# RyanXLi/OneshotDet

Hardware: AMD Instinct MI355X
Metric: images/sec/GPU fwd+bwd, 800x1024 target + 127x127 query, bs=8; 1->8 GPU scaling (higher is better)
Workload: dtype bf16; 1 GPU; BASELINE.json configs[2]: bs=8/GPU, 800x1024 target + 127x127 query, bf16 MFMA convs, forward (two R-50-FPN backbones, query pooling, correlation, FCOS head, training proposals) + FCOS loss + backward (stem/layer1 frozen) + gradient all-reduce + SGD(momentum) + weight repack; global_batch=8, parallelism=dp1: one rank, no collective anywhere in the step, world_size=1

## Files before the change

### oneshotdet_amd/_lib.py

```python
import ctypes as C
import os

_HERE = os.path.dirname(os.path.abspath(__file__))
LIB_PATH = os.environ.get("OSD_LIB_PATH") or os.path.join(_HERE, "lib", "liboneshotdet_hip.so")

OSD_F32, OSD_BF16 = 0, 1
ABI_VERSION = 4
ACT_NONE, ACT_RELU, ACT_EXP_SCALE = 0, 1, 2
RES_NONE, RES_SAME, RES_UP2X, RES_DOWN2X = 0, 1, 2, 3
GN_SPLITS = 64


class ConvDesc(C.Structure):
    _fields_ = [(n, C.c_int32) for n in (
        "dtype", "n", "h", "w", "cin", "in_stride_n", "in_stride_h", "in_stride_w", "ho", "wo", "cout", "r", "s",
        "stride_h", "stride_w", "pad_h", "pad_w", "w_rows", "out_stride", "res_mode", "res_h", "res_w", "res_stride",
        "act")] + [("act_scale", C.c_float), ("relu_in", C.c_int32), ("algo", C.c_int32), ("reserved0", C.c_int32),
                   ("ordered_ws", C.c_void_p), ("ordered_ws_bytes", C.c_int64)]


_p, _i, _f, _i64 = C.c_void_p, C.c_int, C.c_float, C.c_int64

SIGNATURES = {
    "osd_last_error_string": (C.c_char_p, []),
# ... 85 lines not shown
    "osd_box_loss": (_i, [_p, _p, _p, _p, _i, _i, _i, _f, _f, _p, _p, _i, _i, _p]),
    "osd_voc_match": (_i, [_p, _p, _p, _p, _p, _p, _p, _p, _i, _i, _i, _f, _p, _p, _p]),
    "osd_voc_curves": (_i, [_p, _p, _p, _i, _p, _p, _p]),
    "osd_voc_ap": (_i, [_p, _p, _p, _p, _p, _i, _i, _p, _p]),
    "osd_coco_match": (_i, [_p, _p, _p, _p, _p, _p, _i, _i, _i, _p, _i, _p, _i, _p, _p, _p, _p]),
    "osd_groupnorm_act_rois_bwd": (_i, [_p, _p, _p, _p, _p, _p, _p, _p, _p, _i, _i, _i, _i, _f, _f, _i, _i, _i, _i, _p]),
    "osd_rois_sum": (_i, [_p, _p, _i, _i, _i64, _i, _p]),
    "osd_roi_pool_levels_bwd": (_i, [_i, _p, _p, _p, _p, _p, _p, _p, _i, _i, _i, _i, _i, _i, _i, _p]),
    "osd_image_transform": (_i, [_p, _i, _i, _i, _i, _i, _i, _p, _p, _p, _i, _i, _i, _i, _i, _i, _i, _p, _p]),
    "osd_image_transform_workspace_bytes": (_i64, [_i, _i, _i, _i]),
    "osd_image_transform_batch": (_i, [_i, _p, _p, _p, _p, _p, _p, _i, _p, _p, _p, _i, _i, _i, _i, _i, _i, _i, _p, _p]),
}

BOX_CLS_CE, BOX_CLS_FOCAL, BOX_CLS_MSE = 0, 1, 2
SIGNATURES_BOX_MODES = {
    "osd_box_loss_opt": (_i, [_p, _p, _p, _p, _i, _i, _i, _f, _f, _p, _p, _i, _i, _i, _f, _f, _p]),
    "osd_box_decode_opt": (_i, [_p, _p, _p, _p, _p, _p, _p, _i, _i, _i, _i, _p, _f, _f, _p, _f, _i, _i, _p]),
}

BOX_CLS_L1, BOX_CLS_CXE = 3, 4
SOFT_LABEL_DISCRETE, SOFT_LABEL_LINEAR, SOFT_LABEL_TRANS_LINEAR, SOFT_LABEL_TRANS_4TH_LINEAR = 0, 1, 2, 3
SIGNATURES_SOFT_LABELS = {
    "osd_box_match_sample_soft": (_i, [_p, _p, _p, _p, _p, _p, _i, _i, _i, _i, _f, _f, _p, _p, _p, _p, _p, _p, _p, _p, _i, _p, _p, _p]),
    "osd_box_loss_soft": (_i, [_p, _p, _p, _p, _i, _i, _i, _f, _f, _p, _p, _i, _i, _p, _i, _p]),
}

SIGNATURES_NEG_SUPPORT = {
    "osd_box_loss_neg_support": (_i, [_p, _p, _p, _p, _p, _i, _i, _i, _f, _f, _f, _f, _p, _p, _p, _i, _i, _p]),
}

SIGNATURES_SOLVER = {
    "osd_solver_set": (_i, [_p, _f, _i, _p]),
    "osd_sgd_momentum_multi_dev": (_i, [_p, _p, _i, _p, _p, _p, _p, _f, _p]),
    "osd_sgd_momentum_pack_multi_dev": (_i, [_p, _p, _i, _p, _p, _p, _p, _p, _i, _p, _f, _i, _p]),
}

SIGNATURES_CLASS_SWEEP = {
    "osd_class_sweep_group": (_i, []),
    "osd_correlate_levels_sweep": (_i, [_i, _p, _p, _p, _p, _i, _i, _i, _i, _p]),
    "osd_roi_pool_levels_sweep": (_i, [_i, _p, _p, _p, _p, _p, _p, _p, _i, _i, _i, _i, _i, _i, _i, _p, _i, _p]),
}

SIGNATURES_GALLERY = {
    "osd_correlate_levels_gallery": (_i, [_i, _p, _p, _p, _p, _p, _i, _i, _i, _i, _i, _p]),
    "osd_groupnorm_act_rois_gallery": (_i, [_p, _p, _p, _p, _p, _p, _i, _i, _i, _i, _f, _f, _i, _i, _i, _i, _i, _p]),
}

PRED_BWD_BOTH, PRED_BWD_DGRAD, PRED_BWD_WGRAD = 0, 1, 2
SIGNATURES_PRED_BWD = {
    "osd_pred_bwd_workspace_bytes": (_i64, [_i, _p, _p, _p, _i, _i]),
    "osd_conv2d_pred_bwd": (_i, [C.POINTER(ConvDesc), _i, _p, _p, _p, _p, _p, _p, _p, _p, _p, _p, _i, _p]),
}

_lib = None


class OsdError(RuntimeError):
    pass


def load():
    global _lib
    if _lib is not None:
        return _lib
    if not os.path.exists(LIB_PATH):
        raise OsdError("liboneshotdet_hip.so not built (%s missing): run `python -m oneshotdet_amd.build` or "
                       "__graft_entry__.build(); there is no CPU/eager fallback" % LIB_PATH)
    import torch
    lib = C.CDLL(LIB_PATH)
    for name, (res, args) in (list(SIGNATURES.items()) + list(SIGNATURES_BOX_MODES.items()) + list(SIGNATURES_SOFT_LABELS.items())
                              + list(SIGNATURES_NEG_SUPPORT.items()) + list(SIGNATURES_SOLVER.items())
                              + list(SIGNATURES_CLASS_SWEEP.items()) + list(SIGNATURES_GALLERY.items())
                              + list(SIGNATURES_PRED_BWD.items())):
        fn = getattr(lib, name)
        fn.restype = res
        fn.argtypes = args
    if lib.osd_abi_version() != ABI_VERSION:
        raise OsdError("%s reports ABI %d, this binding is written for ABI %d: rebuild it (`python -m oneshotdet_amd.build`)"
                       % (LIB_PATH, lib.osd_abi_version(), ABI_VERSION))
    _lib = lib
    return lib


def check(rc, what=""):
    if rc != 0:
        msg = load().osd_last_error_string()
        err = OsdError("%s failed (%d): %s" % (what, rc, msg.decode() if msg else "?"))
        err.code = rc
        raise err


def call(name, *args):
    lib = load()
    check(getattr(lib, name)(*args), name)
```

### oneshotdet_amd/build.py

```python
import os
import subprocess
import sys

HERE = os.path.dirname(os.path.abspath(__file__))
CSRC = os.path.join(HERE, "csrc")
LIBDIR = os.path.join(HERE, "lib")
TAG = os.environ.get("OSD_BUILD_TAG", "")
LIB = os.path.join(LIBDIR, "liboneshotdet_hip%s.so" % ("_" + TAG if TAG else ""))
SOURCES = ["osd_error.hip", "conv_igemm.hip", "conv_igemm_dma.hip", "conv_igemm_sp.hip", "conv_pred.hip", "conv_pred_bwd.hip", "conv_px.hip", "conv_wgrad.hip", "conv_wgrad_sk.hip", "backward.hip", "groupnorm_onepass.hip", "loss.hip", "elementwise.hip", "proposals.hip", "box_head.hip", "transforms.hip", "box_train.hip", "evaluation.hip", "query_avgpool.hip", "class_sweep.hip", "gallery.hip"]
HIPCC = os.environ.get("HIPCC", "/opt/rocm/bin/hipcc")
FLAGS = ["--offload-arch=gfx950", "-O3", "-fPIC", "-std=c++17", "-Wno-unused-result"] + os.environ.get("OSD_BUILD_FLAGS", "").split()


def _stale(target, deps):
    if not os.path.exists(target):
        return True
    t = os.path.getmtime(target)
    return any(os.path.getmtime(d) > t for d in deps)


def build_library(force=False, verbose=True):
    os.makedirs(LIBDIR, exist_ok=True)
    objdir = os.path.join(LIBDIR, "obj" + ("_" + TAG if TAG else ""))
    os.makedirs(objdir, exist_ok=True)
    headers = sorted(os.path.join(CSRC, f) for f in os.listdir(CSRC) if f.endswith(".h")) + [os.path.join(os.path.dirname(HERE), "include", h) for h in ("oneshotdet_hip.h", "oneshotdet_hip_box_modes.h", "oneshotdet_hip_soft_labels.h", "oneshotdet_hip_neg_support.h", "oneshotdet_hip_solver.h", "oneshotdet_hip_class_sweep.h", "oneshotdet_hip_gallery.h", "oneshotdet_hip_pred_bwd.h")]
    keep = set(src.replace(".hip", ".o") for src in SOURCES)
    for f in os.listdir(objdir):
        if f.endswith(".o") and f not in keep:
            os.remove(os.path.join(objdir, f))
    objs, procs = [], []
    for src in SOURCES:
        s = os.path.join(CSRC, src)
        o = os.path.join(objdir, src.replace(".hip", ".o"))
        objs.append(o)
        if force or _stale(o, [s] + headers):
            cmd = [HIPCC] + FLAGS + ["-c", s, "-o", o]
            if verbose:
                print(" ".join(cmd), flush=True)
            procs.append((src, subprocess.Popen(cmd, stdout=subprocess.PIPE, stderr=subprocess.STDOUT)))
    for src, p in procs:
        out, _ = p.communicate()
        if p.returncode != 0:
            sys.stderr.write(out.decode())
            raise RuntimeError("hipcc failed on %s" % src)
    if force or procs or _stale(LIB, objs):
        cmd = [HIPCC, "--offload-arch=gfx950", "-shared", "-fPIC", "-o", LIB] + objs
        if verbose:
            print(" ".join(cmd), flush=True)
        subprocess.check_call(cmd)
    return LIB


if __name__ == "__main__":
    print(build_library(force="--force" in sys.argv))
```

### oneshotdet_amd/csrc/backward.hip

```cpp
#include "osd_common.h"
#include "conv_params.h"

namespace {

constexpr int kMaxBlocks = 2048;
inline int grid_for(long long work, int threads) {
  long long b = (work + threads - 1) / threads;
  if (b < 1) b = 1;
  return (int)(b > kMaxBlocks ? kMaxBlocks : b);
}

template <typename T> struct Chunk;
template <> struct Chunk<float> {
  static constexpr int N = 4;
  float v[4];
  __device__ __forceinline__ void load(const float* p) {
    const float4 t = *reinterpret_cast<const float4*>(p);
    v[0] = t.x; v[1] = t.y; v[2] = t.z; v[3] = t.w;
  }
  __device__ __forceinline__ void store(float* p) const { *reinterpret_cast<float4*>(p) = make_float4(v[0], v[1], v[2], v[3]); }
};
template <> struct Chunk<__bf16> {
  static constexpr int N = 8;
  float v[8];
  __device__ __forceinline__ void load(const __bf16* p) {
    const bf16x8 t = *reinterpret_cast<const bf16x8*>(p);
#pragma unroll
    for (int i = 0; i < 8; ++i) v[i] = (float)t[i];
  }
  __device__ __forceinline__ void store(__bf16* p) const {
    bf16x8 t;
#pragma unroll
    for (int i = 0; i < 8; ++i) t[i] = (__bf16)v[i];
    *reinterpret_cast<bf16x8*>(p) = t;
  }
};

template <typename T>
__global__ void pack_dgrad_weight_kernel(const float* __restrict__ w, const float* __restrict__ scale, T* __restrict__ dst,
                                         int cout, int cin, int R, int S, int rows, int cout_pad, int src_orsi) {
  const long long total = (long long)rows * R * S * cout_pad;
  for (long long i = blockIdx.x * (long long)blockDim.x + threadIdx.x; i < total; i += (long long)gridDim.x * blockDim.x) {
    const int co = (int)(i % cout_pad);
    long long t = i / cout_pad;
    const int s = (int)(t % S); t /= S;
    const int r = (int)(t % R);
    const int ci = (int)(t / R);
    float v = 0.f;
    if (co < cout && ci < cin) {
      v = src_orsi ? w[(((size_t)co * R + (R - 1 - r)) * S + (S - 1 - s)) * cin + ci]
                   : w[(((size_t)co * cin + ci) * R + (R - 1 - r)) * S + (S - 1 - s)];
      if (scale) v *= scale[co];
    }
    dst[i] = from_f32<T>(v);
// ... 774 lines not shown
#pragma unroll
        for (int e = 0; e < E; ++e) s[e] += live * a[k].v[e] * bb[k].v[e];
      }
    }
  }
  __shared__ float red[256 * 8];
#pragma unroll
  for (int e = 0; e < E; ++e) red[(pl * cch + cc) * E + e] = (pl < lanes) ? s[e] : 0.f;
  __syncthreads();
  for (int ch = threadIdx.x; ch < c; ch += blockDim.x) {
    float t = 0.f;
    for (int l = 0; l < lanes; ++l) t += red[l * c + ch];
    if (p0 < p1) atomicAdd(dq + (size_t)img * c + ch, t);
  }
}
}

extern "C" int osd_correlate_bwd_query_levels(int n_levels, const void* const* gs, const void* const* feats,
                                              float* const* dqs, const int32_t* hws, int n, int c, int dtype, void* stream) {
  const int e = dtype == OSD_BF16 ? 8 : 4;
  if (n_levels < 1 || n_levels > kCorrQLevels || !gs || !feats || !dqs || !hws || c % e || 256 % (c / e) || c > 2048)
    return osd_fail(OSD_ERR_INVALID_ARG, "correlate_bwd_query_levels: bad args");
  if (dtype != OSD_F32 && dtype != OSD_BF16) return osd_fail(OSD_ERR_INVALID_ARG, "correlate_bwd_query_levels: bad dtype");
  if (n == 0) return OSD_OK;
  CorrQLevels L;
  L.n_levels = 0;
  int blocks = 0;
  for (int i = 0; i < n_levels; ++i)
    if (!dqs[i]) return osd_fail(OSD_ERR_INVALID_ARG, "correlate_bwd_query_levels: null dq at level %d", i);
  for (int i = 0; i < n_levels;) {
    int j = i + 1;
    while (j < n_levels && dqs[j] == dqs[j - 1] + (size_t)n * c) ++j;
    hipError_t er = hipMemsetAsync(dqs[i], 0, sizeof(float) * (size_t)n * c * (j - i), OSD_STREAM(stream));
    if (er != hipSuccess) return osd_fail(OSD_ERR_LAUNCH, "correlate_bwd_query_levels: memset failed");
    i = j;
  }
  for (int i = 0; i < n_levels; ++i) {
    if (hws[i] <= 0) continue;
    if (!gs[i] || !feats[i]) return osd_fail(OSD_ERR_INVALID_ARG, "correlate_bwd_query_levels: null tensor at level %d", i);
    int slabs = (hws[i] + 63) / 64;
    if (slabs > 512) slabs = 512;
    const int k = L.n_levels++;
    L.g[k] = gs[i]; L.feat[k] = feats[i]; L.dq[k] = dqs[i]; L.hw[k] = hws[i]; L.slabs[k] = slabs; L.begin[k] = blocks;
    blocks += slabs * n;
  }
  if (L.n_levels == 0) return OSD_OK;
  for (int k = L.n_levels; k < kCorrQLevels; ++k) { L.g[k] = L.g[0]; L.feat[k] = L.feat[0]; L.dq[k] = L.dq[0]; L.hw[k] = 0; L.slabs[k] = 1; L.begin[k] = 0x7fffffff; }
  OSD_DISPATCH_DTYPE(dtype,
      hipLaunchKernelGGL(correlate_bwd_q_levels_kernel<float>, dim3(blocks), dim3(256), 0, OSD_STREAM(stream), L, c),
      hipLaunchKernelGGL(correlate_bwd_q_levels_kernel<__bf16>, dim3(blocks), dim3(256), 0, OSD_STREAM(stream), L, c));
  return osd_check_launch("correlate_bwd_query_levels");
}

extern "C" int osd_roialign_bwd(const float* gy, const float* rois, float* gx, int b, int h, int w, int c, int num_rois,
                                float spatial_scale, int ph, int pw, int sampling_ratio, void* stream) {
  if (!gy || !rois || !gx) return osd_fail(OSD_ERR_INVALID_ARG, "roialign_bwd: null argument");
  hipError_t er = hipMemsetAsync(gx, 0, sizeof(float) * (size_t)b * h * w * c, OSD_STREAM(stream));
  if (er != hipSuccess) return osd_fail(OSD_ERR_LAUNCH, "roialign_bwd: memset failed");
  if (num_rois == 0) return OSD_OK;
  const long long cells = (long long)num_rois * ph * pw;
  if (cells > 0x7fffffffLL) return osd_fail(OSD_ERR_INVALID_ARG, "roialign_bwd: too many cells");
  hipLaunchKernelGGL(roialign_bwd_kernel, dim3((unsigned)cells), dim3(64), 0, OSD_STREAM(stream),
                     gy, rois, gx, h, w, c, num_rois, spatial_scale, ph, pw, sampling_ratio);
  return osd_check_launch("roialign_bwd");
}

extern "C" int osd_query_pool_levels_bwd(int n_levels, const float* const* dqs, const int32_t* hs, const int32_t* ws, const float* scales,
                                         const float* rois, int batch, int shots, int c, int sampling_ratio, float* gx32,
                                         void* const* outs, int dtype, void* stream) {
  if (n_levels < 1 || n_levels > kQPoolLevels || !dqs || !hs || !ws || !scales || !rois || !gx32 || !outs || shots < 1 || c < 1)
    return osd_fail(OSD_ERR_INVALID_ARG, "query_pool_levels_bwd: bad arguments");
  if (batch == 0) return OSD_OK;
  QPoolBwdLevels L;
  L.n_levels = n_levels;
  long long off = 0;
  for (int l = 0; l < kQPoolLevels; ++l) {
    const int j = l < n_levels ? l : 0;
    if (!dqs[j] || !outs[j] || hs[j] < 1 || ws[j] < 1) return osd_fail(OSD_ERR_INVALID_ARG, "query_pool_levels_bwd: bad level %d", j);
    L.dq[l] = dqs[j]; L.out[l] = outs[j]; L.h[l] = hs[j]; L.w[l] = ws[j]; L.scale[l] = scales[j];
    L.begin[l] = off;
    L.gx[l] = gx32 + (l < n_levels ? off : 0);
    if (l < n_levels) off += (long long)batch * shots * hs[j] * ws[j] * c;
  }
  for (int l = n_levels; l <= kQPoolLevels; ++l) L.begin[l] = off;
  hipError_t er = hipMemsetAsync(gx32, 0, sizeof(float) * (size_t)off, OSD_STREAM(stream));
  if (er != hipSuccess) return osd_fail(OSD_ERR_LAUNCH, "query_pool_levels_bwd: memset failed");
  hipLaunchKernelGGL(query_pool_levels_bwd_kernel, dim3(batch * shots, n_levels), dim3(64), 0, OSD_STREAM(stream), L, rois, c, shots, sampling_ratio);
  int rc = osd_check_launch("query_pool_levels_bwd");
  if (rc) return rc;
  const int g = grid_for(off, 256);
  OSD_DISPATCH_DTYPE(dtype,
      hipLaunchKernelGGL(query_pool_levels_cast_kernel<float>, dim3(g), dim3(256), 0, OSD_STREAM(stream), L),
      hipLaunchKernelGGL(query_pool_levels_cast_kernel<__bf16>, dim3(g), dim3(256), 0, OSD_STREAM(stream), L));
  return osd_check_launch("query_pool_levels_cast");
}

extern "C" int osd_shot_mean_bwd(const float* gy, float* gx, int b, int shots, int c, void* stream) {
  if (!gy || !gx || shots < 1) return osd_fail(OSD_ERR_INVALID_ARG, "shot_mean_bwd: bad args");
  hipLaunchKernelGGL(shot_mean_bwd_kernel, dim3(cdiv(b * shots * c, 256)), dim3(256), 0, OSD_STREAM(stream), gy, gx, b, shots, c);
  return osd_check_launch("shot_mean_bwd");
}

extern "C" int osd_cast_f32(const float* src, void* dst, int64_t numel, int dtype, void* stream) {
  if (!src || !dst) return osd_fail(OSD_ERR_INVALID_ARG, "cast_f32: null argument");
  if (numel == 0) return OSD_OK;
  const int g = grid_for(numel, 256);
// ... 500 lines not shown
```

### oneshotdet_amd/ops.py

```python
import ctypes as C
import os

import torch

from . import _lib, spec
from ._lib import (ACT_EXP_SCALE, ACT_NONE, ACT_RELU, GN_SPLITS, OSD_BF16, OSD_F32, RES_DOWN2X, RES_NONE, RES_SAME, RES_UP2X,
                   ConvDesc)

__all__ = ["ACT_NONE", "ACT_RELU", "ACT_EXP_SCALE", "RES_NONE", "RES_SAME", "RES_UP2X", "RES_DOWN2X"]


from . import streams

_stream_handle = streams.raw_handle


def _stream():
    return C.c_void_p(_stream_handle())


from .trace import rec as _rec
from . import trace as _trace


# ... 518 lines not shown
    classes = int(classes)
    if classes < 1:
        raise ValueError("classes must be at least 1, got %d" % classes)
    assert all(x.shape[0] == n and x.shape[-1] == c and x.is_contiguous() for x in xs)
    assert all(q.shape == (n * classes, c) and q.dtype == torch.float32 and q.is_contiguous() for q in qs)
    ys = [torch.empty((n * classes,) + tuple(x.shape[1:]), device=x.device, dtype=x.dtype) for x in xs]
    hws = (C.c_int32 * k)(*[x.shape[1] * x.shape[2] for x in xs])
    _lib.call("osd_correlate_levels_sweep", k, _ptr_array(xs), _ptr_array(qs), _ptr_array(ys), hws, n, classes, c, _dt(xs[0]),
              _stream())
    for x, q, y in zip(xs, qs, ys):
        _rec("correlate_sweep", x=x, q=q, out=y, classes=classes)
    return ys


def correlate_levels_gallery(xs, qs, slots, classes):
    _chk_dev(slots, *xs)
    k = len(xs)
    n, c = xs[0].shape[0], xs[0].shape[-1]
    classes = int(classes)
    if classes < 1:
        raise ValueError("classes must be at least 1, got %d" % classes)
    g = qs[0].shape[0]
    assert all(x.shape[0] == n and x.shape[-1] == c and x.is_contiguous() for x in xs)
    assert all(q.shape == (g, c) and q.dtype == torch.float32 and q.is_contiguous() for q in qs)
    assert slots.dtype == torch.int32 and slots.shape == (n * classes,) and slots.is_contiguous()
    ys = [torch.empty((n * classes,) + tuple(x.shape[1:]), device=x.device, dtype=x.dtype) for x in xs]
    if n == 0:
        return ys
    hws = (C.c_int32 * k)(*[x.shape[1] * x.shape[2] for x in xs])
    _lib.call("osd_correlate_levels_gallery", k, _ptr_array(xs), _ptr_array(qs), _p(slots), _ptr_array(ys), hws, n, classes, g, c,
              _dt(xs[0]), _stream())
    for x, q, y in zip(xs, qs, ys):
        _rec("correlate_gallery", x=x, q=q, slots=slots, out=y, classes=classes)
    return ys


def class_sweep_group():
    return int(_lib.load().osd_class_sweep_group())


def correlate_bwd_query_levels(gs, feats):
    k = len(gs)
    n, c = gs[0].shape[0], gs[0].shape[-1]
    dq = torch.empty((k, n, c), device=gs[0].device, dtype=torch.float32)
    dqs = [dq[l] for l in range(k)]
    hws = (C.c_int32 * k)(*[g.shape[1] * g.shape[2] for g in gs])
    _lib.call("osd_correlate_bwd_query_levels", k, _ptr_array(gs), _ptr_array(feats), _ptr_array(dqs), hws, n, c, _dt(gs[0]),
              _stream())
    for g, f, o in zip(gs, feats, dqs):
        _rec("correlate_bwd_query", g=g, feat=f, out=o)
    return dqs


def nhwc_to_nchw_f32(x, c0=0, c=None):
    _chk_dev(x)
    n, h, w, stride = x.shape
    c = stride - c0 if c is None else c
    y = torch.empty((n, c, h, w), device=x.device, dtype=torch.float32)
    _lib.call("osd_nhwc_to_nchw_f32", _p(x), _p(y), n, h, w, c, stride, c0, _dt(x), _stream())
    return y


def nchw_f32_to_nhwc(x, dtype):
    _chk_dev(x)
    n, c, h, w = x.shape
    y = torch.empty((n, h, w, c), device=x.device, dtype=dtype)
    _lib.call("osd_nchw_f32_to_nhwc", _ptr(x.contiguous().float()), _p(y), n, c, h, w, _dt(y), _stream())
    return y


def fcos_score_decode(cls_ctr, reg, scores, boxes, stride, loc_offset, img_h, img_w, img_hw=None):
    _chk_dev(cls_ctr, reg, scores, boxes, img_hw)
    n, h, w, ccs = cls_ctr.shape
    _lib.call("osd_fcos_score_decode_sizes", _p(cls_ctr), _p(reg), _p(scores), _p(boxes), n, h, w, ccs,
              reg.shape[-1], stride, loc_offset, scores.shape[1], float(img_h), float(img_w), _p(img_hw), _dt(cls_ctr),
              _stream())


def level_topk(keys, lo, cnt, topn):
    n, total = keys.shape
    _lib.call("osd_level_topk", _p(keys), _p(keys), n, total, lo, cnt, topn, _stream())


def rank_sort_gather(keys, boxes, max_count, levels=None, topn=0):
    _chk_dev(keys, boxes)
    n, total = keys.shape
    dev = keys.device
    bs = torch.empty((n, max_count, 4), device=dev, dtype=torch.float32)
    ss = torch.empty((n, max_count), device=dev, dtype=torch.float32)
    idx = torch.empty((n, max_count), device=dev, dtype=torch.int32)
    cnt = torch.empty((n,), device=dev, dtype=torch.int32)
    if levels:
        lo = (C.c_int32 * len(levels))(*[l for l, _ in levels])
        lc = (C.c_int32 * len(levels))(*[c for _, c in levels])
        nl = len(levels)
    else:
        lo, lc, nl = None, None, 0
    _lib.call("osd_rank_sort_gather", _p(keys), _p(boxes), n, total, max_count, lo, lc, nl, int(topn), _p(bs),
              _p(ss), _p(idx), _p(cnt), _stream())
    return bs, ss, idx, cnt


def nms_sorted(boxes_sorted, scores_sorted, counts, thresh, max_keep, cuda_semantics=False, workspace=None):
    _chk_dev(boxes_sorted, scores_sorted, counts)
    n, max_count, _ = boxes_sorted.shape
    dev = boxes_sorted.device
# ... 813 lines not shown
```

### oneshotdet_amd/train.py

```python
import math
import os

import torch

from . import streams

from . import ops, spec

from .train_backward import BackwardPass
from .train_forward import SIZE_RANGES, ForwardPass
from .train_second_stage import SecondStage
from .train_state import State
from .train_update import Update


def _payload(t):
    from .layers import ImageList
    if isinstance(t, ops.PackedImages):
        return t.tensor
    if isinstance(t, ImageList):
        return t.tensors
    return t


# ... 45 lines not shown
        self.wstream = torch.cuda.Stream(device=self.device) if wgrad_side_stream else None
        self.s1 = torch.cuda.Stream(device=self.device) if wgrad_side_stream else None
        self.wstream2 = torch.cuda.Stream(device=self.device) if wgrad_side_stream else None
        self.pstream = torch.cuda.Stream(device=self.device) if wgrad_side_stream else None
        self._keep = []
        self.second_stage = bool(second_stage)
        self.box_keys, self.box_losses = None, None
        self.box_suppress_loss = None
        from .model import ProposalDepth
        self._prop_depth = None if os.environ.get("OSD_NO_PROP_HINT") else ProposalDepth()
        self.lockstep = os.environ.get("OSD_LOCKSTEP", "0") != "0"
        self.corr_levels = os.environ.get("OSD_CORR_LEVELS", "1") != "0"
        self.skip_unused_c2 = os.environ.get("OSD_FULL_C2", "0") == "0"
        self.towers_merged = os.environ.get("OSD_TOWERS_MERGED", "0") != "0"
        self.split_levels = os.environ.get("OSD_SPLIT_LEVELS", "0") != "0"
        self.fuse_head_sum = os.environ.get("OSD_NO_HEAD_SUM_FUSION", "0") == "0"
        if not self.siamese_backbone:
            self.BBS = ("backbone.", "backbone.")
        self._shared_held = {}
        sd = {k: torch.as_tensor(v).to(self.device, torch.float32) for k, v in state_dict.items()
              if self.siamese_backbone or not spec.is_query_backbone_key(k)}
        missing = [k for k in spec.hot_path_shapes(self.siamese_backbone) if k not in sd]
        if missing:
            raise KeyError("state_dict is missing hot-path keys (siamese_backbone=%r), e.g. %s" % (self.siamese_backbone, missing[:3]))
        self._frozen_sd = sd
        self.convs = {}
        self.extra = {}
        self._plan = []
        self._build(sd)
        self._allocate(sd)
        from . import model as _model
        self._fused_l1 = {}
        if _model.FUSE_DOWNSAMPLE and dtype == torch.bfloat16:
            for bb in dict.fromkeys(self.BBS):
                if (bb + "body.layer1.0.downsample.0.weight") in sd:
                    self._fused_l1[bb] = _model.pack_conv3_downsample(sd, bb + "body.layer1.0.", dtype)
        from .dist_utils import GradExchange, bucket_ranges
        self.ustream = torch.cuda.Stream(device=self.device)
        for pair in [a for a in os.environ.get("OSD_STREAM_ALIAS", "").split(",") if "=" in a]:
            names = {"w": "wstream", "w2": "wstream2", "s1": "s1", "p": "pstream", "u": "ustream"}
            dst, src = pair.split("=")
            if getattr(self, names[src]) is not None:
                setattr(self, names[dst], getattr(self, names[src]))
        self.exchange = GradExchange(self.flat_g, bucket_ranges(self._plan, self.flat_g.numel()), self.pg,
                                     single_rank_too=exchange_single_rank, wire_dtype=grad_wire_dtype, comm_stream=self.ustream)
        self._overlap, self._fuse_update, self._updated = True, False, set()
        self.consume_grads = os.environ.get("OSD_NO_CONSUME_GRADS", "0") == "0"
        self._grads_clean, self._zeroed = False, set()
        self._wqs = None
        self._pred_grad_bufs = {}
        self.pred_dgrad_gemm = os.environ.get("OSD_NO_PRED_DGRAD_GEMM", "0") == "0"
        self._pred_dgrad = {}
        self.pred_bwd_fused = os.environ.get("OSD_PRED_BWD_FUSED", "1") != "0"
        self.tower_wgrad_at = os.environ.get("OSD_TOWER_WGRAD_AT", "")
        self._held_wgrads = []
        if ordered_wgrad is None:
            ordered_wgrad = os.environ.get("OSD_WGRAD_ORDERED", "0") != "0"
        self.ordered_wgrad = bool(ordered_wgrad)
        self.fuse_gn_bwd = (not self.ordered_wgrad and self.dtype == torch.bfloat16 and os.environ.get("OSD_GN_FUSION", "0") != "0")
        self._gnb_ws = {}
        self.fpn_out_grouped = os.environ.get("OSD_NO_FPN_GROUPED", "0") == "0"
        self.gn_conv_db = (not self.ordered_wgrad and os.environ.get("OSD_NO_GN_CONV_DB", "0") == "0" and not ops.GN_ONEPASS_BWD)
        self.fuse_gn_fwd = (not self.ordered_wgrad and self.dtype == torch.bfloat16 and os.environ.get("OSD_GN_FWD_FUSION", "0") != "0")
        self._gnf_ws = {}
        cands = (self.wstream, self.wstream2) + ((self.pstream,) if self.second_stage else ())
        self._wgrad_streams = list({id(x): x for x in cands if x is not None}.values()) or [streams.current()]
        if self.ordered_wgrad and self.second_stage:
            import warnings
            warnings.warn("ordered_wgrad makes every conv_wgrad launch bit-reproducible, the second stage's included; its "
                          "ROI-pool backward (osd_roi_pool_levels_bwd) still scatters with fp32 atomics, so the gradients it "
                          "feeds into both backbones are reproducible only up to the order of those adds")
        for st in self._wgrad_streams:
            ops.wgrad_set_workspace(st, (1 << 30) if self.ordered_wgrad else 0)
        if self.wstream is not None:
            self.warm_streams()
        self.defer_join = False
        self._deferred, self._defer_now, self._joined_refs = None, False, None
        self.repack()
        self.zero_bias = torch.zeros(4096, device=self.device, dtype=torch.float32)
        weights = [c.w for c in self.convs.values() if c.trainable] + \
                  [p for n, (p, _) in self.extra.items() if "bias" not in n]
        biases = [c.b for c in self.convs.values() if c.trainable and c.has_bias] + \
                 [p for n, (p, _) in self.extra.items() if "bias" in n]
        self.lr, self.momentum, self.weight_decay = lr, momentum, weight_decay
        self.lr_schedule, self._solver, self._dev_update = lr_schedule, None, False
        self.opt = None
        if optimizer == "torch":
            self.opt = torch.optim.SGD([{"params": weights, "lr": lr, "weight_decay": weight_decay},
                                        {"params": biases, "lr": 2 * lr, "weight_decay": 0.0}], lr=lr, momentum=momentum)
            self._sgd = dict(tables={}, buf=None, steps=0)
        else:
            self._build_sgd_table(weights, biases)

    def _add_conv(self, name, sd, bn=None, bias=None, trainable=True):
        w = sd[name + ".weight"]
        cout, cin, r, s = w.shape
        c = TConv(name, cout, cin, r, s, trainable, bias is not None)
        if bn is not None:
            g, b, mean, var = (sd[bn + k] for k in (".weight", ".bias", ".running_mean", ".running_var"))
            c.bn_scale = (g * var.rsqrt()).contiguous()
            c.bn_shift = (b - mean * c.bn_scale).contiguous()
        self.convs[name] = c
        if trainable:
            self._plan.append((name + ".weight", (cout, r, s, cin)))
            if bias is not None:
                self._plan.append((name + ".bias", (cout,)))
# ... 199 lines not shown
        af = join_previous if deferred is not None else None

        def pool(qf):
            if not self.supp_roialign:
                return ops.query_avgpool_levels(qf, batch)
            if ops.QUERY_POOL_LEVELS and len(qf) <= 8:
                return ops.query_pool_levels(qf, rois, spec.POOLER_SCALES, batch, spec.POOLER_SAMPLING_RATIO)
            out = []
            for feat, scale in zip(qf, spec.POOLER_SCALES):
                v = ops.roi_align(feat, rois, scale, 1, 1, spec.POOLER_SAMPLING_RATIO)
                out.append(ops.shot_mean(v.view(v.shape[0], -1), batch))
            return out
        if lock:
            (feats, qfeats), (tctx, qctx) = self.backbones_forward(images, qin, after_frozen=af)
            qfeats, nqfeats, qfeats_all = self._split_neg_rows(qfeats, batch)
            pooled = pool(qfeats)
        else:
            if deferred is not None and s1 is not None:
                for ev in deferred["events"]:
                    s1.wait_event(ev)
            side.wait_stream(main)
            if s1 is None and af is not None:
                af()
                af = None
            with streams.on(side):
                (qfeats,), (qctx,) = self._backbones_forward(self.BBS[1:], (qin,))
                qfeats, nqfeats, qfeats_all = self._split_neg_rows(qfeats, batch)
                pooled = pool(qfeats)
            (feats,), (tctx,) = self._backbones_forward(self.BBS[:1], (images,), af)
            main.wait_stream(side)
        prev_keep = deferred = self._joined_refs = None
        combined = ops.correlate_levels(feats, pooled) if self.corr_levels else [ops.correlate(f, q) for f, q in zip(feats, pooled)]
        head_out, hctx = self.head_forward(combined)
        if with_proposals:
            ps = self.pstream if self.pstream is not None else main
            if ps is not main:
                ps.wait_stream(main)
            with streams.on(ps):
                pb, ps_, pc = model.run_proposals(head_out, images.shape[-2], images.shape[-1],
                                                  spec.PRE_NMS_TOP_N_TRAIN, spec.POST_NMS_TOP_N_TRAIN, spec.NMS_THRESH,
                                                  image_sizes=image_sizes,
                                                  depth=self._prop_depth)
                self.proposals = ops.append_gt_boxes(pb, ps_, pc, gt_boxes, gt_count)
                if self.second_stage:
                    neg_kw = dict(neg_qfeats=nqfeats, neg_q_sizes=nq_sizes) if self.neg_support else {}
                    box_out = self.box_head_forward_backward(feats, qfeats, q_sizes, shots, self.proposals, gt_boxes, gt_count,
                                                             keys=self.box_keys, **neg_kw)
                    self._bucket_ready("box_head", 0, [ps])
        losses, pred_grads = self.loss_and_grads(head_out, gt_boxes, gt_count)
        self.last_head_out, self.last_pred_grads = head_out, pred_grads
        d_comb = self.head_backward(combined, hctx, pred_grads)
        if not self._held_wgrads:
            self._bucket_ready("head", 0, [st for st in (main, self.wstream, self.wstream2) if st is not None])
        dq = ops.correlate_bwd_query_levels(d_comb, feats) if self.corr_levels else \
            [ops.correlate_bwd_query(g, f) for g, f in zip(d_comb, feats)]
        second = self.second_stage and with_proposals
        ps = self.pstream if self.pstream is not None else main
        if s1 is not None:
            s1.wait_stream(main)
            if second and ps is not main:
                s1.wait_stream(ps)
        if second:
            if ps is not main:
                main.wait_stream(ps)
            if self.neg_support:
                box5, gx, gqs, gqs_neg = box_out
                self.box_losses, self.box_suppress_loss = box5[:3], box5[3:]
            else:
                self.box_losses, gx, gqs = box_out
        with streams.on(side):
            dQ = []
            if not self.supp_roialign:
                dQ = ops.query_avgpool_levels_bwd(dq, [tuple(qf.shape) for qf in qfeats], shots, self.dtype)
            elif ops.QUERY_POOL_LEVELS and len(dq) <= 8:
                dQ = ops.query_pool_levels_bwd(dq, rois, [tuple(qf.shape) for qf in qfeats], spec.POOLER_SCALES, shots,
                                               spec.POOLER_SAMPLING_RATIO, self.dtype)
            else:
                for dql, qf, scale in zip(dq, qfeats, spec.POOLER_SCALES):
                    dv = ops.shot_mean_bwd(dql, shots)
                    gxq = ops.roi_align_bwd(dv.view(-1, 1, 1, dv.shape[-1]), rois, qf.shape, scale, 1, 1,
                                            spec.POOLER_SAMPLING_RATIO)
                    dQ.append(ops.cast_f32(gxq, self.dtype))
            if second:
                for lvl, gq in gqs:
                    if shots > 1:
                        full = torch.zeros((gq.shape[0] * shots,) + tuple(gq.shape[1:]), device=self.device, dtype=torch.float32)
                        full[::shots] = gq
                        gq = full
                    dQ[lvl] = ops.add_mask(dQ[lvl], ops.cast_f32(gq, self.dtype))
            if self.neg_support:
                full = [torch.zeros(tuple(qa.shape), device=self.device, dtype=self.dtype) for qa in qfeats_all]
                for l, d in enumerate(dQ):
                    ops.add_mask(d, None, None, out=full[l][:batch])
                if second:
                    for lvl, gq in gqs_neg:
                        ops.add_mask(ops.cast_f32(gq, self.dtype), None, None, out=full[lvl][batch:])
                self._keep.append((dQ, qfeats_all))
                dQ = full
            if not lock:
                self.backbones_backward([qctx], [dQ], which0=1)
        dP = ops.correlate_levels(d_comb, pooled) if self.corr_levels else [ops.correlate(g, q) for g, q in zip(d_comb, pooled)]
        if second:
            dP = [ops.add_mask(d, ops.cast_f32(g, self.dtype)) for d, g in zip(dP, gx)]
            self._keep.append((gx, gqs, gqs_neg if self.neg_support else None))
        if lock:
            if s1 is not None:
                main.wait_stream(s1)
            self.backbones_backward([tctx, qctx], [dP, dQ])
        else:
            self.backbones_backward([tctx], [dP])
        self._keep.append((dq, dP, dQ, d_comb, pred_grads))
        if self._defer_now:
            events = []
            for st in (s1, self.wstream, self.wstream2, self.pstream, self.ustream, self.exchange.comm):
                if st is not None:
                    ev = torch.cuda.Event()
                    ev.record(st)
                    events.append(ev)
            self._deferred = dict(events=events, refs=(qctx, tctx, hctx, feats, qfeats, qfeats_all, pooled, combined, head_out, dQ, rois))
            return losses
        if s1 is not None:
            main.wait_stream(s1)
        if self.wstream is not None:
            main.wait_stream(self.wstream)
        if self.wstream2 is not None:
            main.wait_stream(self.wstream2)
        if with_proposals and self.pstream is not None:
            main.wait_stream(self.pstream)
        return losses

    def _split_neg_rows(self, qfeats, batch):
        if not self.neg_support:
            return qfeats, None, qfeats
        return [f[:batch] for f in qfeats], [f[batch:] for f in qfeats], qfeats

    def join(self):
        d, self._deferred = self._deferred, None
        if d is not None:
            cur = streams.current()
            for ev in d["events"]:
                cur.wait_event(ev)
            self._joined_refs = d["refs"]

    def reduce_gradients(self):
        self.exchange.finish()

    @property
    def iteration(self):
        return self._sgd["steps"]

    def _scheduled_lr(self):
        if self.lr_schedule is None:
            return
        self.lr = self.lr_schedule.lr_at(self.iteration)
# ... 73 lines not shown
```

Before: 792.0 images/sec.

## Fuse correlation backward dP and dq into one multi-level kernel with deferred fold

```diff
diff --git a/include/oneshotdet_hip_head_tail.h b/include/oneshotdet_hip_head_tail.h
--- /dev/null
+++ b/include/oneshotdet_hip_head_tail.h
@@ -0,0 +1,28 @@
+#ifndef ONESHOTDET_HIP_HEAD_TAIL_H
+#define ONESHOTDET_HIP_HEAD_TAIL_H
+
+#include "oneshotdet_hip.h"
+
+#ifdef __cplusplus
+extern "C" {
+#endif
+
+#define OSD_CORR_BWD_FOLD_INLINE 0
+#define OSD_CORR_BWD_FOLD_DEFERRED 1
+
+int64_t osd_correlate_bwd_levels_workspace_bytes(int n_levels, const int32_t* hws, int n, int c);
+
+int64_t osd_correlate_bwd_levels_sync_bytes(int n_levels, int n);
+
+int osd_correlate_bwd_levels(int n_levels, const void* const* gs, const void* const* feats, const float* const* qs, void* const* dps,
+                             float* const* dqs, const int32_t* hws, int n, int c, int dtype, void* workspace, void* sync, int flags,
+                             void* stream);
+
+int osd_correlate_bwd_levels_fold(int n_levels, float* const* dqs, const int32_t* hws, int n, int c, const void* workspace,
+                                  void* stream);
+
+#ifdef __cplusplus
+}
+#endif
+
+#endif
diff --git a/oneshotdet_amd/_lib.py b/oneshotdet_amd/_lib.py
--- a/oneshotdet_amd/_lib.py
+++ b/oneshotdet_amd/_lib.py
@@ -161,6 +161,14 @@
     "osd_conv2d_pred_bwd": (_i, [C.POINTER(ConvDesc), _i, _p, _p, _p, _p, _p, _p, _p, _p, _p, _p, _i, _p]),
 }
 
+CORR_BWD_FOLD_INLINE, CORR_BWD_FOLD_DEFERRED = 0, 1
+SIGNATURES_HEAD_TAIL = {
+    "osd_correlate_bwd_levels_workspace_bytes": (_i64, [_i, _p, _i, _i]),
+    "osd_correlate_bwd_levels_sync_bytes": (_i64, [_i, _i]),
+    "osd_correlate_bwd_levels": (_i, [_i, _p, _p, _p, _p, _p, _p, _i, _i, _i, _p, _p, _i, _p]),
+    "osd_correlate_bwd_levels_fold": (_i, [_i, _p, _p, _i, _i, _p, _p]),
+}
+
 _lib = None
 
 
@@ -180,7 +188,7 @@
     for name, (res, args) in (list(SIGNATURES.items()) + list(SIGNATURES_BOX_MODES.items()) + list(SIGNATURES_SOFT_LABELS.items())
                               + list(SIGNATURES_NEG_SUPPORT.items()) + list(SIGNATURES_SOLVER.items())
                               + list(SIGNATURES_CLASS_SWEEP.items()) + list(SIGNATURES_GALLERY.items())
-                              + list(SIGNATURES_PRED_BWD.items())):
+                              + list(SIGNATURES_PRED_BWD.items()) + list(SIGNATURES_HEAD_TAIL.items())):
         fn = getattr(lib, name)
         fn.restype = res
         fn.argtypes = args
diff --git a/oneshotdet_amd/build.py b/oneshotdet_amd/build.py
--- a/oneshotdet_amd/build.py
+++ b/oneshotdet_amd/build.py
@@ -23,7 +23,7 @@
     os.makedirs(LIBDIR, exist_ok=True)
     objdir = os.path.join(LIBDIR, "obj" + ("_" + TAG if TAG else ""))
     os.makedirs(objdir, exist_ok=True)
-    headers = sorted(os.path.join(CSRC, f) for f in os.listdir(CSRC) if f.endswith(".h")) + [os.path.join(os.path.dirname(HERE), "include", h) for h in ("oneshotdet_hip.h", "oneshotdet_hip_box_modes.h", "oneshotdet_hip_soft_labels.h", "oneshotdet_hip_neg_support.h", "oneshotdet_hip_solver.h", "oneshotdet_hip_class_sweep.h", "oneshotdet_hip_gallery.h", "oneshotdet_hip_pred_bwd.h")]
+    headers = sorted(os.path.join(CSRC, f) for f in os.listdir(CSRC) if f.endswith(".h")) + [os.path.join(os.path.dirname(HERE), "include", h) for h in ("oneshotdet_hip.h", "oneshotdet_hip_box_modes.h", "oneshotdet_hip_soft_labels.h", "oneshotdet_hip_neg_support.h", "oneshotdet_hip_solver.h", "oneshotdet_hip_class_sweep.h", "oneshotdet_hip_gallery.h", "oneshotdet_hip_pred_bwd.h", "oneshotdet_hip_head_tail.h")]
     keep = set(src.replace(".hip", ".o") for src in SOURCES)
     for f in os.listdir(objdir):
         if f.endswith(".o") and f not in keep:
diff --git a/oneshotdet_amd/csrc/backward.hip b/oneshotdet_amd/csrc/backward.hip
--- a/oneshotdet_amd/csrc/backward.hip
+++ b/oneshotdet_amd/csrc/backward.hip
@@ -1,5 +1,6 @@
 #include "osd_common.h"
 #include "conv_params.h"
+#include "../../include/oneshotdet_hip_head_tail.h"
 
 namespace {
 
@@ -880,6 +881,234 @@
   return osd_check_launch("correlate_bwd_query_levels");
 }
 
+constexpr int kCorrBLevels = 6;
+constexpr int kCorrBMaxC = 1024;
+struct CorrBwdLevels {
+  const void* g[kCorrBLevels]; const void* feat[kCorrBLevels]; const float* q[kCorrBLevels];
+  void* dp[kCorrBLevels]; float* dq[kCorrBLevels];
+  int hw[kCorrBLevels], slabs[kCorrBLevels], begin[kCorrBLevels];
+  int n_levels;
+};
+namespace {
+__device__ __forceinline__ void corr_bwd_fold_slots(const float* base, int slabs, int c, int ch0, int cw, float* red, float* out) {
+  const int tpr = cw / 4, ngr = 256 / tpr;
+  const int cq = threadIdx.x % tpr, gr = threadIdx.x / tpr;
+  const float* src0 = base + ch0 + cq * 4;
+  float acc[4] = {0.f, 0.f, 0.f, 0.f};
+  constexpr int V = 16;
+  for (int sl = gr; sl < slabs; sl += V * ngr) {
+    float4 v[V];
+#pragma unroll
+    for (int k = 0; k < V; ++k) v[k] = *reinterpret_cast<const float4*>(src0 + (size_t)min(sl + k * ngr, slabs - 1) * c);
+#pragma unroll
+    for (int k = 0; k < V; ++k) {
+      const bool on = sl + k * ngr < slabs;
+      acc[0] += on ? v[k].x : 0.f; acc[1] += on ? v[k].y : 0.f; acc[2] += on ? v[k].z : 0.f; acc[3] += on ? v[k].w : 0.f;
+    }
+  }
+#pragma unroll
+  for (int j = 0; j < 4; ++j) red[gr * cw + cq * 4 + j] = acc[j];
+  __syncthreads();
+  for (int ch = threadIdx.x; ch < cw; ch += blockDim.x) {
+    float t = 0.f;
+    for (int r = 0; r < ngr; ++r) t += red[r * cw + ch];
+    out[ch0 + ch] = t;
+  }
+}
+
+__host__ __device__ inline int corr_bwd_fold_width(int c) { return (c % 64 == 0) ? 64 : c; }
+
+template <typename T, bool INLINE_FOLD>
+__global__ void __launch_bounds__(256) correlate_bwd_levels_kernel(CorrBwdLevels L, float* ws, int* __restrict__ cnt, int n, int c) {
+  constexpr int E = Chunk<T>::N;
+  __shared__ float red[256 * 8];
+  __shared__ float qs[kCorrBMaxC];
+  __shared__ int last_flag;
+  const int b = blockIdx.x;
+  int lvl = 0;
+#pragma unroll
+  for (int i = 1; i < kCorrBLevels; ++i)
+    if (i < L.n_levels && b >= L.begin[i]) lvl = i;
+  const void* gv = L.g[0]; const void* fv = L.feat[0]; const float* q = L.q[0]; void* dpv = L.dp[0]; float* dq = L.dq[0];
+  int hw = L.hw[0], slabs = L.slabs[0], beg = L.begin[0];
+#pragma unroll
+  for (int i = 1; i < kCorrBLevels; ++i)
+    if (lvl == i) { gv = L.g[i]; fv = L.feat[i]; q = L.q[i]; dpv = L.dp[i]; dq = L.dq[i]; hw = L.hw[i]; slabs = L.slabs[i]; beg = L.begin[i]; }
+  const T* g = reinterpret_cast<const T*>(gv);
+  const T* feat = reinterpret_cast<const T*>(fv);
+  T* dp = reinterpret_cast<T*>(dpv);
+  const int local = b - beg;
+  const int img = local / slabs, slab = local - img * slabs;
+  for (int i = threadIdx.x; i < c; i += blockDim.x) qs[i] = q[(size_t)img * c + i];
+  __syncthreads();
+  const int cch = c / E;
+  const int lanes = 256 / cch;
+  const int cc = threadIdx.x % cch, pl = threadIdx.x / cch;
+  const int per = (hw + slabs - 1) / slabs;
+  const int p0 = slab * per, p1 = min(hw, p0 + per);
+  float s[E], qv[E];
+#pragma unroll
+  for (int e = 0; e < E; ++e) { s[e] = 0.f; qv[e] = qs[cc * E + e]; }
+  if (pl < lanes && p0 < p1) {
+    constexpr int U = 4;
+    for (int p = p0 + pl; p < p1; p += U * lanes) {
+      Chunk<T> a[U], bb[U];
+#pragma unroll
+      for (int k = 0; k < U; ++k) {
+        const size_t off = ((size_t)img * hw + min(p + k * lanes, p1 - 1)) * c + cc * E;
+        a[k].load(g + off);
+        bb[k].load(feat + off);
+      }
+#pragma unroll
+      for (int k = 0; k < U; ++k) {
+        const bool on = p + k * lanes < p1;
+        const float live = on ? 1.f : 0.f;
+#pragma unroll
+        for (int e = 0; e < E; ++e) s[e] += live * a[k].v[e] * bb[k].v[e];
+        if (on) {
+          Chunk<T> o;
+#pragma unroll
+          for (int e = 0; e < E; ++e) o.v[e] = a[k].v[e] * qv[e];
+          o.store(dp + ((size_t)img * hw + p + k * lanes) * c + cc * E);
+        }
+      }
+    }
+  }
+#pragma unroll
+  for (int e = 0; e < E; ++e) red[(pl * cch + cc) * E + e] = (pl < lanes) ? s[e] : 0.f;
+  __syncthreads();
+  for (int ch = threadIdx.x; ch < c; ch += blockDim.x) {
+    float t = 0.f;
+    for (int l = 0; l < lanes; ++l) t += red[l * c + ch];
+    if (INLINE_FOLD) __hip_atomic_store(ws + (size_t)b * c + ch, t, __ATOMIC_RELAXED, __HIP_MEMORY_SCOPE_AGENT);
+    else ws[(size_t)b * c + ch] = t;
+  }
+  if (!INLINE_FOLD) return;
+  asm volatile("s_waitcnt vmcnt(0)" ::: "memory");
+  __syncthreads();
+  if (threadIdx.x == 0) {
+    int* a = cnt + (lvl * n + img);
+    const int last = __hip_atomic_fetch_add(a, 1, __ATOMIC_RELAXED, __HIP_MEMORY_SCOPE_AGENT) == slabs - 1;
+    if (last) {
+      __hip_atomic_store(a, 0, __ATOMIC_RELAXED, __HIP_MEMORY_SCOPE_AGENT);
+      __builtin_amdgcn_fence(__ATOMIC_ACQUIRE, "agent");
+      asm volatile("s_waitcnt vmcnt(0)" ::: "memory");
+    }
+    last_flag = last;
+  }
+  __syncthreads();
+  if (!last_flag) return;
+  const int cw = corr_bwd_fold_width(c);
+  for (int ch0 = 0; ch0 < c; ch0 += cw) {
+    corr_bwd_fold_slots(ws + (size_t)(beg + img * slabs) * c, slabs, c, ch0, cw, red, dq + (size_t)img * c);
+    __syncthreads();
+  }
+}
+
+struct CorrBwdFold {
+  float* dq[kCorrBLevels];
+  int slabs[kCorrBLevels], begin[kCorrBLevels];
+};
+__global__ void __launch_bounds__(256) correlate_bwd_fold_kernel(CorrBwdFold F, const float* __restrict__ ws, int n, int c, int cw) {
+  __shared__ float red[1024];
+  const int lvl = blockIdx.x / n, img = blockIdx.x - lvl * n;
+  float* dq = F.dq[0];
+  int slabs = F.slabs[0], beg = F.begin[0];
+#pragma unroll
+  for (int i = 1; i < kCorrBLevels; ++i)
+    if (lvl == i) { dq = F.dq[i]; slabs = F.slabs[i]; beg = F.begin[i]; }
+  corr_bwd_fold_slots(ws + (size_t)(beg + img * slabs) * c, slabs, c, blockIdx.y * cw, cw, red, dq + (size_t)img * c);
+}
+
+inline int corr_bwd_slabs(int hw) {
+  const int s = (hw + 63) / 64;
+  return s > 512 ? 512 : s;
+}
+inline bool corr_bwd_c_ok(int c, int dtype) {
+  const int e = dtype == OSD_BF16 ? 8 : 4;
+  return c > 0 && c <= kCorrBMaxC && c % e == 0 && 256 % (c / e) == 0 && 256 % (c / 4) == 0;
+}
+}
+
+extern "C" int64_t osd_correlate_bwd_levels_workspace_bytes(int n_levels, const int32_t* hws, int n, int c) {
+  if (n_levels < 1 || n_levels > kCorrBLevels || !hws || n < 0 || !corr_bwd_c_ok(c, OSD_F32)) return 0;
+  int64_t blocks = 0;
+  for (int i = 0; i < n_levels; ++i)
+    if (hws[i] > 0) blocks += (int64_t)corr_bwd_slabs(hws[i]) * n;
+  return blocks * c * (int64_t)sizeof(float);
+}
+
+extern "C" int64_t osd_correlate_bwd_levels_sync_bytes(int n_levels, int n) {
+  if (n_levels < 1 || n_levels > kCorrBLevels || n < 0) return 0;
+  return (int64_t)n_levels * n * (int64_t)sizeof(int);
+}
+
+extern "C" int osd_correlate_bwd_levels(int n_levels, const void* const* gs, const void* const* feats, const float* const* qs,
+                                        void* const* dps, float* const* dqs, const int32_t* hws, int n, int c, int dtype,
+                                        void* workspace, void* sync, int flags, void* stream) {
+  if (dtype != OSD_F32 && dtype != OSD_BF16) return osd_fail(OSD_ERR_INVALID_ARG, "correlate_bwd_levels: bad dtype");
+  if (flags != OSD_CORR_BWD_FOLD_INLINE && flags != OSD_CORR_BWD_FOLD_DEFERRED)
+    return osd_fail(OSD_ERR_INVALID_ARG, "correlate_bwd_levels: bad flags %d", flags);
+  const bool inl = flags == OSD_CORR_BWD_FOLD_INLINE;
+  if (n_levels < 1 || n_levels > kCorrBLevels || !gs || !feats || !qs || !dps || (inl && !dqs) || !hws || n < 0 || !corr_bwd_c_ok(c, dtype))
+    return osd_fail(OSD_ERR_INVALID_ARG, "correlate_bwd_levels: bad args");
+  if (n == 0) return OSD_OK;
+  CorrBwdLevels L;
+  L.n_levels = 0;
+  long long blocks = 0;
+  for (int i = 0; i < n_levels; ++i) {
+    if (hws[i] <= 0) continue;
+    if (!gs[i] || !feats[i] || !qs[i] || !dps[i] || (inl && !dqs[i]))
+      return osd_fail(OSD_ERR_INVALID_ARG, "correlate_bwd_levels: null tensor at level %d", i);
+    const int k = L.n_levels++;
+    L.g[k] = gs[i]; L.feat[k] = feats[i]; L.q[k] = qs[i]; L.dp[k] = dps[i]; L.dq[k] = inl ? dqs[i] : nullptr;
+    L.hw[k] = hws[i]; L.slabs[k] = corr_bwd_slabs(hws[i]); L.begin[k] = (int)blocks;
+    blocks += (long long)L.slabs[k] * n;
+    if (blocks > 0x7ffffff0LL) return osd_fail(OSD_ERR_INVALID_ARG, "correlate_bwd_levels: too many workgroups");
+  }
+  if (L.n_levels == 0) return OSD_OK;
+  if (!workspace || (inl && !sync)) return osd_fail(OSD_ERR_INVALID_ARG, "correlate_bwd_levels: null workspace");
+  for (int k = L.n_levels; k < kCorrBLevels; ++k) {
+    L.g[k] = L.g[0]; L.feat[k] = L.feat[0]; L.q[k] = L.q[0]; L.dp[k] = L.dp[0]; L.dq[k] = L.dq[0];
+    L.hw[k] = 0; L.slabs[k] = 1; L.begin[k] = 0x7fffffff;
+  }
+  const dim3 grid((unsigned)blocks);
+  if (inl) {
+    OSD_DISPATCH_DTYPE(dtype,
+        hipLaunchKernelGGL((correlate_bwd_levels_kernel<float, true>), grid, dim3(256), 0, OSD_STREAM(stream), L, (float*)workspace, (int*)sync, n, c),
+        hipLaunchKernelGGL((correlate_bwd_levels_kernel<__bf16, true>), grid, dim3(256), 0, OSD_STREAM(stream), L, (float*)workspace, (int*)sync, n, c));
+  } else {
+    OSD_DISPATCH_DTYPE(dtype,
+        hipLaunchKernelGGL((correlate_bwd_levels_kernel<float, false>), grid, dim3(256), 0, OSD_STREAM(stream), L, (float*)workspace, (int*)nullptr, n, c),
+        hipLaunchKernelGGL((correlate_bwd_levels_kernel<__bf16, false>), grid, dim3(256), 0, OSD_STREAM(stream), L, (float*)workspace, (int*)nullptr, n, c));
+  }
+  return osd_check_launch("correlate_bwd_levels");
+}
+
+extern "C" int osd_correlate_bwd_levels_fold(int n_levels, float* const* dqs, const int32_t* hws, int n, int c, const void* workspace,
+                                             void* stream) {
+  if (n_levels < 1 || n_levels > kCorrBLevels || !dqs || !hws || n < 0 || !corr_bwd_c_ok(c, OSD_F32))
+    return osd_fail(OSD_ERR_INVALID_ARG, "correlate_bwd_levels_fold: bad args");
+  if (n == 0) return OSD_OK;
+  CorrBwdFold F;
+  int k = 0;
+  long long blocks = 0;
+  for (int i = 0; i < n_levels; ++i) {
+    if (hws[i] <= 0) continue;
+    if (!dqs[i]) return osd_fail(OSD_ERR_INVALID_ARG, "correlate_bwd_levels_fold: null dq at level %d", i);
+    F.dq[k] = dqs[i]; F.slabs[k] = corr_bwd_slabs(hws[i]); F.begin[k] = (int)blocks;
+    blocks += (long long)F.slabs[k] * n;
+    ++k;
+  }
+  if (k == 0) return OSD_OK;
+  if (!workspace) return osd_fail(OSD_ERR_INVALID_ARG, "correlate_bwd_levels_fold: null workspace");
+  for (int j = k; j < kCorrBLevels; ++j) { F.dq[j] = F.dq[0]; F.slabs[j] = 1; F.begin[j] = 0; }
+  const int cw = corr_bwd_fold_width(c);
+  hipLaunchKernelGGL(correlate_bwd_fold_kernel, dim3((unsigned)(k * n), (unsigned)(c / cw)), dim3(256), 0, OSD_STREAM(stream), F,
+                     (const float*)workspace, n, c, cw);
+  return osd_check_launch("correlate_bwd_levels_fold");
+}
+
 extern "C" int osd_roialign_bwd(const float* gy, const float* rois, float* gx, int b, int h, int w, int c, int num_rois,
                                 float spatial_scale, int ph, int pw, int sampling_ratio, void* stream) {
   if (!gy || !rois || !gx) return osd_fail(OSD_ERR_INVALID_ARG, "roialign_bwd: null argument");
diff --git a/oneshotdet_amd/ops.py b/oneshotdet_amd/ops.py
--- a/oneshotdet_amd/ops.py
+++ b/oneshotdet_amd/ops.py
@@ -594,6 +594,55 @@
     return dqs
 
 
+_CORR_BWD_SYNC = {}
+
+
+def correlate_bwd_levels_ok(gs):
+    c = gs[0].shape[-1]
+    e = 8 if gs[0].dtype == torch.bfloat16 else 4
+    return 1 <= len(gs) <= 6 and 0 < c <= 1024 and c % e == 0 and 256 % (c // e) == 0 and 256 % (c // 4) == 0
+
+
+def _corr_bwd_sync(dev, k, n):
+    key = (dev.index, _stream_handle())
+    buf = _CORR_BWD_SYNC.get(key)
+    if buf is None or buf.numel() < k * n:
+        buf = _CORR_BWD_SYNC[key] = torch.zeros((max(k * n, 64),), device=dev, dtype=torch.int32)
+    return buf
+
+
+def correlate_bwd_levels(gs, feats, qs, ws=None, sync=None, deferred=False):
+    _chk_dev(*gs)
+    k = len(gs)
+    n, c = gs[0].shape[0], gs[0].shape[-1]
+    assert all(g.shape[0] == n and g.shape[-1] == c and g.is_contiguous() and f.shape == g.shape and f.is_contiguous() and
+               f.dtype == g.dtype for g, f in zip(gs, feats))
+    assert all(q.shape == (n, c) and q.dtype == torch.float32 and q.is_contiguous() for q in qs)
+    dev = gs[0].device
+    dps = [torch.empty_like(g) for g in gs]
+    dq = torch.empty((k, n, c), device=dev, dtype=torch.float32)
+    dqs = [dq[l] for l in range(k)]
+    hws = (C.c_int32 * k)(*[g.shape[1] * g.shape[2] for g in gs])
+    if ws is None:
+        need = int(_lib.load().osd_correlate_bwd_levels_workspace_bytes(k, hws, n, c))
+        ws = torch.empty((need // 4 + 1,), device=dev, dtype=torch.float32)
+    if sync is None and not deferred:
+        sync = _corr_bwd_sync(dev, k, n)
+    _lib.call("osd_correlate_bwd_levels", k, _ptr_array(gs), _ptr_array(feats), _ptr_array(qs), _ptr_array(dps),
+              None if deferred else _ptr_array(dqs), hws, n, c, _dt(gs[0]), _p(ws), None if deferred else _p(sync),
+              _lib.CORR_BWD_FOLD_DEFERRED if deferred else _lib.CORR_BWD_FOLD_INLINE, _stream())
+    for g, q, y in zip(gs, qs, dps):
+        _rec("correlate", x=g, q=q, out=y)
+
+    def fold():
+        if deferred:
+            _lib.call("osd_correlate_bwd_levels_fold", k, _ptr_array(dqs), hws, n, c, _p(ws), _stream())
+        for g, f, o in zip(gs, feats, dqs):
+            _rec("correlate_bwd_query", g=g, feat=f, out=o)
+        return dqs
+    return (dps, fold) if deferred else (dps, fold())
+
+
 def nhwc_to_nchw_f32(x, c0=0, c=None):
     _chk_dev(x)
     n, h, w, stride = x.shape
diff --git a/oneshotdet_amd/train.py b/oneshotdet_amd/train.py
--- a/oneshotdet_amd/train.py
+++ b/oneshotdet_amd/train.py
@@ -121,6 +121,10 @@
         self.pred_dgrad_gemm = os.environ.get("OSD_NO_PRED_DGRAD_GEMM", "0") == "0"
         self._pred_dgrad = {}
         self.pred_bwd_fused = os.environ.get("OSD_PRED_BWD_FUSED", "1") != "0"
+        self.head_tail = os.environ.get("OSD_HEAD_TAIL", "1") != "0"
+        self.head_tail_fold = os.environ.get("OSD_HEAD_TAIL_FOLD", "launch")
+        if self.head_tail_fold not in ("launch", "inline"):
+            raise ValueError("OSD_HEAD_TAIL_FOLD must be launch or inline, got %r" % self.head_tail_fold)
         self.tower_wgrad_at = os.environ.get("OSD_TOWER_WGRAD_AT", "")
         self._held_wgrads = []
         if ordered_wgrad is None:
@@ -426,8 +430,15 @@
         d_comb = self.head_backward(combined, hctx, pred_grads)
         if not self._held_wgrads:
             self._bucket_ready("head", 0, [st for st in (main, self.wstream, self.wstream2) if st is not None])
-        dq = ops.correlate_bwd_query_levels(d_comb, feats) if self.corr_levels else \
-            [ops.correlate_bwd_query(g, f) for g, f in zip(d_comb, feats)]
+        dP = dq_fold = None
+        if self.corr_levels and self.head_tail and ops.correlate_bwd_levels_ok(d_comb):
+            dP, dq = ops.correlate_bwd_levels(d_comb, feats, pooled, deferred=self.head_tail_fold == "launch")
+            if callable(dq):
+                dq_fold, dq = dq, None
+                self._keep.append(dq_fold)
+        else:
+            dq = ops.correlate_bwd_query_levels(d_comb, feats) if self.corr_levels else \
+                [ops.correlate_bwd_query(g, f) for g, f in zip(d_comb, feats)]
         second = self.second_stage and with_proposals
         ps = self.pstream if self.pstream is not None else main
         if s1 is not None:
@@ -443,6 +454,8 @@
             else:
                 self.box_losses, gx, gqs = box_out
         with streams.on(side):
+            if dq_fold is not None:
+                dq = dq_fold()
             dQ = []
             if not self.supp_roialign:
                 dQ = ops.query_avgpool_levels_bwd(dq, [tuple(qf.shape) for qf in qfeats], shots, self.dtype)
@@ -473,7 +486,8 @@
                 dQ = full
             if not lock:
                 self.backbones_backward([qctx], [dQ], which0=1)
-        dP = ops.correlate_levels(d_comb, pooled) if self.corr_levels else [ops.correlate(g, q) for g, q in zip(d_comb, pooled)]
+        if dP is None:
+            dP = ops.correlate_levels(d_comb, pooled) if self.corr_levels else [ops.correlate(g, q) for g, q in zip(d_comb, pooled)]
         if second:
             dP = [ops.add_mask(d, ops.cast_f32(g, self.dtype)) for d, g in zip(dP, gx)]
             self._keep.append((gx, gqs, gqs_neg if self.neg_support else None))
```

Result: no change. 791.0 images/sec (-0.1%).
